# hbdat/cvpr22_cross_modal_pseudo_labeling

Hardware: AMD Instinct MI355X
Metric: images/sec student-teacher train step (COCO 800x1333) (higher is better)
Workload: dtype f32 (bf16x3 split MFMA, fp32 accum); 1 GPU; student_teacher_mask_rcnn_uncertainty.yaml R-50-C4, 2 img/GPU 3x800x1333, fwd+bwd+allreduce+SGD; global_batch=2, parallelism=dp1, losses_finite=True, pipelined=True

## Files before the change

cvpr22_cross_modal_pseudo_labeling_amd/_C.py:

```python
import contextlib
import functools
import ctypes
import threading

import torch

from . import _cpu, _lib

_L = _lib.load()


def _stream():
    return torch._C._cuda_getCurrentRawStream(torch.cuda.current_device())


class _Same:

    def __enter__(self):
        return None

    def __exit__(self, *exc):
        return False


# ... 652 lines not shown
        if not (pooled.is_cuda and pooled.dtype == torch.float32 and pooled.dim() == 2):
            raise RuntimeError("gate_split_pair: pooled must be a 2-D float32 HIP tensor")
        pooled = pooled.contiguous()
    if dy is not None:
        if not (dy.is_cuda and dy.dtype == torch.float32 and dy.dim() == 2):
            raise RuntimeError("gate_split_pair: 2-D float32 HIP tensor expected")
        if dy.stride(1) != 1 or dy.stride(0) % 4 or dy.data_ptr() % 16:
            dy = dy.contiguous()
        rows, cols = dy.shape
    else:
        rows, cols = pooled.shape[0] * pool_rows, pooled.shape[1]
    if pooled is not None and (pool_rows <= 0 or pooled.shape != (rows // max(pool_rows, 1), cols) or rows % pool_rows):
        raise RuntimeError("gate_split_pair: pooled must be [rows / pool_rows, cols]")
    dev = dy.device if dy is not None else pooled.device
    is_pair = 0
    if gate is not None:
        is_pair = int(gate.dtype == torch.bfloat16)
        if not (gate.is_cuda and gate.is_contiguous() and gate.shape == (rows, cols * (2 if is_pair else 1))
                and gate.dtype in (torch.bfloat16, torch.float32)):
            raise RuntimeError("gate_split_pair: gate must be the contiguous fp32 or pair form of the forward output")
    out = torch.empty((rows, 2 * cols), dtype=torch.bfloat16, device=dev)
    g32 = torch.empty((rows, cols), dtype=torch.float32, device=dev) if want_f32 else None
    if out.numel() == 0:
        return out, g32
    if selected is not None:
        selected, group_slot = _dev(selected, "selected"), _dev(group_slot, "group_slot", torch.int32)
        if pool_rows <= 0 or rows % pool_rows or selected.dim() != 2 or selected.shape[1] != cols or \
                selected.shape[0] % pool_rows or group_slot.numel() != rows // pool_rows:
            raise RuntimeError("gate_split_pair: selected must be [S * pool_rows, cols] and group_slot [rows / pool_rows]")
    with _on(dev):
        rc = _L.ovis_gate_split_pair_rows_f32(0 if dy is None else dy.data_ptr(), 0 if dy is None else dy.stride(0),
# ... 161 lines not shown
    if m == 0 or n == 0:
        return c, cp, pooled
    if bias is not None:
        bias = _dev(bias, "bias")
    with _on(dev):
        rc = _L.ovis_split_gemm_pair_rp_pool(a_pair.data_ptr(), 2 * a_pair.stride(0), b_pair.data_ptr(), 2 * b_pair.stride(0),
                                             0 if c is None else c.data_ptr(), n, 0 if cp is None else cp.data_ptr(), 4 * n,
                                             0 if bias is None else bias.data_ptr(),
                                             0 if residual_pair is None else residual_pair.data_ptr(),
                                             0 if residual_pair is None else 2 * residual_pair.stride(0), m, n, ch,
                                             int(bool(relu)), pooled.data_ptr(), int(pool_rows), 1.0 / pool_rows, _stream())
    _lib.check(rc, "split_gemm_pair_rp_pool")
    return c, cp, pooled


def weight_prep_pair(w, scale=None, want_transposed=False):
    if not (w.is_cuda and w.dtype == torch.float32 and w.dim() == 4):
        raise RuntimeError("weight_prep_pair: [N,C,KH,KW] float32 HIP tensor expected")
    w = w.detach().contiguous()
    n, c, kh, kw = w.shape
    t = kh * kw
    fwd = torch.empty((n, 2 * t * c), dtype=torch.bfloat16, device=w.device)
    bwd = torch.empty((c, 2 * t * n), dtype=torch.bfloat16, device=w.device) if want_transposed else None
    if scale is not None:
        scale = _dev(scale.detach(), "scale")
    with _on(w.device):
        rc = _L.ovis_weight_prep_pair_f32(w.data_ptr(), 0 if scale is None else scale.data_ptr(), fwd.data_ptr(),
                                          0 if bwd is None else bwd.data_ptr(), n, c, t, _stream())
    _lib.check(rc, "weight_prep_pair")
    return fwd, bwd
# ... 511 lines not shown
```

cvpr22_cross_modal_pseudo_labeling_amd/_lib.py:

```python
import ctypes
import os

_HERE = os.path.dirname(os.path.abspath(__file__))
LIB_PATH = os.path.join(_HERE, "libovis_hip.so")

OVIS_OK = 0
_ERRORS = {-1: "OVIS_EINVAL (bad size or null pointer)",
           -2: "OVIS_ENOSPC (workspace too small)",
           -3: "OVIS_ERANGE (problem size not supported by the kernel)"}

_vp, _i, _f, _sz, _l = ctypes.c_void_p, ctypes.c_int, ctypes.c_float, ctypes.c_size_t, ctypes.c_long

SIGNATURES = {
    "ovis_version": (ctypes.c_char_p, []),
    "ovis_roi_align_forward_f32": (_i, [_vp, _vp, _vp, _i, _i, _i, _i, _i, _i, _i, _f, _i, _vp]),
    "ovis_roi_align_forward_workspace_bytes": (_sz, [_i, _i, _i]),
    "ovis_roi_align_forward_mfma_supported": (_i, [_i, _i, _i, _i]),
    "ovis_roi_align_forward_ws_f32": (_i, [_vp, _vp, _vp, _i, _i, _i, _i, _i, _i, _i, _f, _i, _vp, _sz, _vp]),
    "ovis_roi_align_forward_strided_nhwc_f32": (_i, [_vp, _vp, _vp, _i, _i, _i, _i, _i, _i, _i, _i, _f, _i, _vp]),
    "ovis_roi_align_forward_strided_pair_f32": (_i, [_vp, _vp, _vp, _i, _i, _i, _i, _i, _i, _i, _i, _f, _i, _vp]),
    "ovis_roi_align_forward_strided_from_nhwc_f32": (_i, [_vp, _vp, _vp, _i, _i, _i, _i, _i, _i, _i, _i, _f, _i, _i, _vp]),
    "ovis_roi_align_backward_f32": (_i, [_vp, _vp, _vp, _i, _i, _i, _i, _i, _i, _i, _f, _i, _vp]),
    "ovis_roi_align_backward_workspace_bytes": (_sz, [_i, _i, _i, _i]),
    "ovis_roi_align_backward_plane_supported": (_i, [_i, _i, _i, _i]),
# ... 29 lines not shown
    "ovis_gate_split_pair_rows_f32": (_i, [_vp, _l, _vp, _i, _vp, _vp, _l, _i, _vp, _i, _vp, _vp, _vp]),
    "ovis_gate_split_pair_f32": (_i, [_vp, _l, _vp, _i, _vp, _vp, _l, _i, _vp, _i, _vp]),
    "ovis_im2col_nchw_pair_f32": (_i, [_vp, _vp] + [_i] * 9 + [_vp]),
    "ovis_weight_prep_pair_f32": (_i, [_vp, _vp, _vp, _vp, _i, _i, _i, _vp]),
    "ovis_slab_reduce_f32": (_i, [_vp, _vp, _vp, _i, _i, _i, _i, _vp]),
    "ovis_im2col_pair": (_i, [_vp, _vp, _l, _i, _i, _i, _i, _i, _vp]),
    "ovis_split_gemm_tn_slices": (_i, [_l, _i, _i, _i]),
    "ovis_split_gemm_pair_tn": (_i, [_vp, _l, _vp, _l, _vp, _i, _l, _i, _i, _i, _i, _i, _i, _vp]),
    "ovis_split_gemm_pair_gated": (_i, [_vp, _l, _vp, _l, _vp, _l, _vp, _l, _vp, _l, _l] + [_i] * 8 + [_vp]),
    "ovis_split_gemm_pair_gated_ws": (_i, [_vp, _l, _vp, _l, _vp, _l, _vp, _l, _vp, _l, _l] + [_i] * 7 + [_vp, _sz, _i, _vp]),
    "ovis_split_gemm_pair_workspace_bytes": (_sz, [_l, _i, _i, _i, _i, _i, _i]),
    "ovis_split_gemm_pair_workspace_bytes_ex": (_sz, [_l, _i, _i, _i, _i, _i, _i, _i]),
    "ovis_split_gemm_pair_rp_gated": (_i, [_vp, _l, _vp, _l, _vp, _l, _vp, _l, _vp, _l, _vp, _l, _l, _i, _i, _i, _vp]),
    "ovis_split_gemm_pair_pool_supported": (_i, [_l, _i, _i, _i]),
    "ovis_split_gemm_pair_rp_pool": (_i, [_vp, _l, _vp, _l, _vp, _l, _vp, _l, _vp, _vp, _l, _l, _i, _i, _i, _vp, _i, _f, _vp]),
    "ovis_split_gemm_pair_rp": (_i, [_vp, _l, _vp, _l, _vp, _l, _vp, _l, _vp, _vp, _l, _l, _i, _i, _i, _vp, _sz, _i, _vp]),
    "ovis_split_gemm_pair": (_i, [_vp, _l, _vp, _l, _vp, _l, _vp, _l, _vp, _l, _vp, _vp, _l, _l] + [_i] * 9
                             + [_vp, _sz, _i, _vp]),
    "ovis_match_encode_f32": (_i, [_vp, _vp, _vp, _i, _i, _f, _f, _i, _f, _f, _f, _f, _vp, _vp, _vp, _vp]),
    "ovis_rpn_match_encode_f32": (_i, [_vp, _vp, _vp, _i, _i, _f, _f, _i, _f, _f, _f, _f, _vp, _vp, _vp, _vp]),
    "ovis_project_masks_f32": (_i, [_vp, _vp, _vp, _i, _i, _i, _i, _i, _vp, _vp]),
    "ovis_gemm_f32": (_i, [_vp, _l, _l, _vp, _l, _l, _vp, _vp, _l, _i, _i, _i, _vp]),
    "ovis_gemm_ex_f32": (_i, [_vp, _l, _l, _vp, _l, _l, _vp, _i, _f, _i, _vp, _l, _i, _i, _i, _vp]),
    "ovis_gemm_f32_workspace_bytes": (_sz, [_i, _i, _i]),
    "ovis_gemm_ex_ws_f32": (_i, [_vp, _l, _l, _vp, _l, _l, _vp, _i, _f, _i, _vp, _l, _i, _i, _i, _vp, _sz, _vp]),
    "ovis_deform_im2col_f32": (_i, [_vp, _vp, _vp, _vp] + [_i] * 13 + [_vp]),
    "ovis_deform_col2im_f32": (_i, [_vp, _vp, _vp, _vp] + [_i] * 13 + [_vp]),
    "ovis_deform_col2im_coord_f32": (_i, [_vp, _vp, _vp, _vp, _vp, _vp] + [_i] * 13 + [_vp]),
    "ovis_deform_im2col_pair_rows_f32": (_i, [_vp, _vp, _vp, _vp, _l] + [_i] * 15 + [_vp]),
    "ovis_deform_col2im_rows_f32": (_i, [_vp, _l, _vp, _vp, _vp, _vp, _vp, _vp] + [_i] * 15 + [_vp]),
# ... 40 lines not shown
```

cvpr22_cross_modal_pseudo_labeling_amd/csrc/split_gemm.hip:

```cpp
#include <stdlib.h>

#include "ovis_common.h"
constexpr int kGroupWidth = 4;

namespace {
typedef short bf16x8 __attribute__((ext_vector_type(8)));
typedef float f32x4 __attribute__((ext_vector_type(4)));
typedef __bf16 b2 __attribute__((ext_vector_type(2)));
typedef float f2 __attribute__((ext_vector_type(2)));

__device__ char g_zero_line[128];

enum { PLAIN = 0, SHIFTED = 1, HALO = 2, DEFORM = 3 };
constexpr int kHalo = 8;

struct SplitGemmArgs {
  const char* A; long a_rs;
  const char* A2; long a2_rs;
  const char* B; long b_rs;
  float* C; long ldc;
  char* Cp; long cp_rs;
  const float* bias; const float* res; long ldr;
  const char* resp; long resp_rs;
  const char* gate; long gate_rs;
  float* pool; int pool_rows; float pool_scale;
  float* slab;
  long M; int N; int ch; int ch2; int T; int H; int W; int KH; int KW; int flip; int relu; int gw;
  int kslices; int steps_per_slice;
  const float* dimg; const float* doff; const float* dmask;
  int Ho; int Wo; int sh; int sw; int ph; int pw; int dlh; int dlw; int dg;
};

__device__ __forceinline__ void glds16(const char* gsrc, char* lds_wave_base) {
  __builtin_amdgcn_global_load_lds((const __attribute__((address_space(1))) void*)gsrc,
                                   (__attribute__((address_space(3))) void*)lds_wave_base, 16, 0, 0);
}

__device__ __forceinline__ unsigned pack_bf16(float a, float b) {
  f2 v = {a, b};
  return __builtin_bit_cast(unsigned, __builtin_convertvector(v, b2));
}

struct EpilogueOperands {
  uint2 a, b;
};

struct EpilogueSource {
  const char* base;
  long row_bytes;
  int second;
};

__device__ __forceinline__ EpilogueSource epilogue_source(const SplitGemmArgs& p) {
  EpilogueSource s;
  s.base = p.res ? (const char*)p.res : (p.resp ? p.resp : p.gate);
// ... 44 lines not shown
    *(uint2*)(d + 64) = make_uint2(l01, l23);
  }
  return v;
}

__device__ __forceinline__ void epilogue_store4(const SplitGemmArgs& p, long m, int n, f32x4 v) {
  const long poff = (long)(n >> 5) * 128 + (n & 31) * 2;
  f32x4 bias4 = {0.f, 0.f, 0.f, 0.f};
  if (p.bias) bias4 = *(const f32x4*)(p.bias + n);
  const EpilogueSource src = epilogue_source(p);
  EpilogueOperands o;
  if (src.base) epilogue_fetch4(src, m, epilogue_column_bytes(p, n, poff), o);
  epilogue_apply4(p, m, n, poff, v, bias4, o);
}

template <int WM, int WN, int MODE, int NS, int OCC, bool DUAL = false, bool POOL = false>
__global__ __launch_bounds__(WM * WN * 64, OCC) void split_gemm_kernel(SplitGemmArgs p, int tiles_n, int ntiles) {
  constexpr int BM = WM * 64, BN = WN * 64, NW = WM * WN;
  constexpr int A_ROWS = MODE == HALO ? BM + 2 * kHalo + 2 : BM;
  constexpr int ZROW = BM + 2 * kHalo;
  constexpr int A_BYTES = A_ROWS * 128, B_BYTES = BN * 128, STAGE = A_BYTES + B_BYTES;
  constexpr int A_PIECES = (MODE == HALO ? BM + 2 * kHalo : BM) / 8;
  constexpr int AI = (A_PIECES + NW - 1) / NW;
  constexpr int BI = BN / 8 / NW;
  static_assert(MODE != HALO || NS == 1, "the halo tile is single-staged");
  static_assert(NW * 4096 <= STAGE * NS, "epilogue staging fits the k-loop's LDS");
  extern __shared__ __attribute__((aligned(16))) char smem[];

  const int lane = threadIdx.x & 63, wave = __builtin_amdgcn_readfirstlane(threadIdx.x >> 6);
  int id;
  {
// ... 316 lines not shown
      const long m = m0 + wm * 64 + (piece >> 1) * 16 + ((piece & 1) * 2 + j) * 4 + er;
      const long mc = m < m_last ? m : m_last;
      epilogue_fetch4(src, mc, src_col, o[j]);
      if constexpr (DUAL) g[j] = *(const uint2*)(gate_col + mc * p.gate_rs);
    }
  };
  f32x4 ps0 = {0.f, 0.f, 0.f, 0.f}, ps1 = ps0, ps2 = ps0;
  int pool_b1 = 0, pool_b2 = 0;
  long pool_map0 = 0;
  if constexpr (POOL) {
    const long mw = m0 + wm * 64;
    pool_map0 = mw / p.pool_rows;
    pool_b1 = (int)((pool_map0 + 1) * p.pool_rows - mw);
    pool_b2 = pool_b1 + p.pool_rows;
  }
#pragma unroll
  for (int i = 0; i < NBUF - 1; ++i) fetch(i, ops[i], gates[i]);
#pragma unroll
  for (int f = 0; f < 4; ++f) {
#pragma unroll
    for (int g = 0; g < 4; ++g) *(f32x4*)(stg + frow * 256 + (((g * 4 + fc) ^ frow) << 4)) = acc[f][g];
#pragma unroll
    for (int h = 0; h < 2; ++h) {
      const int piece = f * 2 + h;
      if (piece + NBUF - 1 < 8) fetch(piece + NBUF - 1, ops[(piece + NBUF - 1) % NBUF], gates[(piece + NBUF - 1) % NBUF]);
#pragma unroll
      for (int j = 0; j < 2; ++j) {
        const int r = (h * 2 + j) * 4 + er;
        const f32x4 v = *(const f32x4*)(stg + r * 256 + ((es ^ r) << 4));
        const long m = m0 + wm * 64 + f * 16 + r;
        if (m < p.M && col_ok) {
          if (slab) *(f32x4*)(slab + m * p.N + n) = v;
          else {
            const f32x4 fin = epilogue_apply4<DUAL>(p, m, n, poff, v, bias4, ops[piece % NBUF][j], gates[piece % NBUF][j]);
            if constexpr (POOL) {
              const int rr = f * 16 + r;
              const f32x4 z = {0.f, 0.f, 0.f, 0.f};
              ps0 += rr < pool_b1 ? fin : z;
              ps1 += (rr >= pool_b1 && rr < pool_b2) ? fin : z;
              ps2 += rr >= pool_b2 ? fin : z;
            }
          }
        }
      }
    }
  }
  if constexpr (POOL) {
    f32x4* ps[3] = {&ps0, &ps1, &ps2};
#pragma unroll
    for (int sgm = 0; sgm < 3; ++sgm) {
      f32x4 v = *ps[sgm];
#pragma unroll
      for (int e = 0; e < 4; ++e) {
        v[e] += __shfl_xor(v[e], 16, 64);
        v[e] += __shfl_xor(v[e], 32, 64);
      }
      const long first = (m0 + wm * 64) + (sgm == 0 ? 0 : (sgm == 1 ? pool_b1 : pool_b2));
// ... 233 lines not shown
    const long r = i / oc;
    const int c = (int)(i - r * oc) * 8;
    const float4 v0 = *(const float4*)(src + r * src_rs + c), v1 = *(const float4*)(src + r * src_rs + c + 4);
    const unsigned h0 = pack_bf16(v0.x, v0.y), h1 = pack_bf16(v0.z, v0.w), h2 = pack_bf16(v1.x, v1.y),
                   h3 = pack_bf16(v1.z, v1.w);
    const unsigned l0 = pack_bf16(v0.x - __uint_as_float(h0 << 16), v0.y - __uint_as_float(h0 & 0xffff0000u));
    const unsigned l1 = pack_bf16(v0.z - __uint_as_float(h1 << 16), v0.w - __uint_as_float(h1 & 0xffff0000u));
    const unsigned l2 = pack_bf16(v1.x - __uint_as_float(h2 << 16), v1.y - __uint_as_float(h2 & 0xffff0000u));
    const unsigned l3 = pack_bf16(v1.z - __uint_as_float(h3 << 16), v1.w - __uint_as_float(h3 & 0xffff0000u));
    char* d = dst + r * 4L * cols + (long)(c >> 5) * 128 + (c & 31) * 2;
    *(uint4*)d = make_uint4(h0, h1, h2, h3);
    *(uint4*)(d + 64) = make_uint4(l0, l1, l2, l3);
  }
}

template <bool GATE_PAIR, bool WRITE_F32>
__global__ __launch_bounds__(256) void gate_split_pair_kernel(const float* __restrict__ dy, long dy_rs,
                                                             const void* __restrict__ gate, char* __restrict__ dst,
                                                             float* __restrict__ g32, long rows, int cols,
                                                             const float* __restrict__ gpool, int pool_rows,
                                                             float pool_scale, const float* __restrict__ gsel,
                                                             const int* __restrict__ group_slot) {
  const int oc = cols >> 3;
  const long total = rows * oc;
  for (long i = (long)blockIdx.x * 256 + threadIdx.x; i < total; i += (long)gridDim.x * 256) {
    const long r = i / oc;
    const int c = (int)(i - r * oc) * 8;
    float v[8];
    if (dy) {
      *(float4*)v = *(const float4*)(dy + r * dy_rs + c);
      *(float4*)(v + 4) = *(const float4*)(dy + r * dy_rs + c + 4);
// ... 11 lines not shown
    }
    if (gsel) {
      const long grp = r / pool_rows;
      const int slot = group_slot[grp];
      if (slot >= 0) {
        const float* gs = gsel + ((long)slot * pool_rows + (r - grp * pool_rows)) * cols + c;
        float q[8];
        *(float4*)q = *(const float4*)gs;
        *(float4*)(q + 4) = *(const float4*)(gs + 4);
#pragma unroll
        for (int k = 0; k < 8; ++k) v[k] += q[k];
      }
    }
    const long poff = r * 4L * cols + (long)(c >> 5) * 128 + (c & 31) * 2;
    if (gate) {
      if (GATE_PAIR) {
        const uint4 h = *(const uint4*)((const char*)gate + poff);
        const unsigned w[4] = {h.x, h.y, h.z, h.w};
#pragma unroll
        for (int k = 0; k < 4; ++k) {
          const unsigned a = w[k] & 0xffffu, b = w[k] >> 16;
          if (a == 0u || a >= 0x8000u) v[2 * k] = 0.f;
          if (b == 0u || b >= 0x8000u) v[2 * k + 1] = 0.f;
        }
      } else {
        float y[8];
        *(float4*)y = *(const float4*)((const float*)gate + r * (long)cols + c);
        *(float4*)(y + 4) = *(const float4*)((const float*)gate + r * (long)cols + c + 4);
#pragma unroll
        for (int k = 0; k < 8; ++k)
          if (!(y[k] > 0.f)) v[k] = 0.f;
// ... 169 lines not shown
                                       pool_rows, nullptr, nullptr, stream);
}

extern "C" int ovis_gate_split_pair_rows_f32(const float* dy, long dy_row_stride, const void* gate, int gate_is_pair,
                                             void* dst_pair, float* g_f32, long rows, int cols, const float* g_pooled,
                                             int pool_rows, const float* g_selected, const int32_t* group_slot,
                                             void* stream) {
  if (rows < 0 || cols < 0) return OVIS_EINVAL;
  if (rows == 0 || cols == 0) return OVIS_OK;
  if ((!dy && !g_pooled && !g_selected) || !dst_pair || ((g_pooled || g_selected) && (pool_rows <= 0 || rows % pool_rows != 0)) ||
      ((g_selected != nullptr) != (group_slot != nullptr)))
    return OVIS_EINVAL;
  if (cols % 32 != 0 || dy_row_stride % 4 != 0 || ((uintptr_t)dy & 15) || ((uintptr_t)dst_pair & 15) ||
      ((uintptr_t)gate & 15) || ((uintptr_t)g_f32 & 15) || ((uintptr_t)g_pooled & 15) || ((uintptr_t)g_selected & 15))
    return OVIS_ERANGE;
  const float pool_scale = g_pooled ? 1.f / (float)pool_rows : 0.f;
  const long total = rows * (cols / 8);
  const long blocks = (total + 255) / 256;
  const unsigned grid = (unsigned)(blocks < 8L * OVIS_NUM_CU ? blocks : 8L * OVIS_NUM_CU);
  hipStream_t s = (hipStream_t)stream;
#define OVIS_GS(GP_, WF_)                                                                                          \
  hipLaunchKernelGGL((gate_split_pair_kernel<GP_, WF_>), dim3(grid), dim3(256), 0, s, dy, dy_row_stride, gate,      \
                     (char*)dst_pair, g_f32, rows, cols, g_pooled, pool_rows, pool_scale, g_selected, group_slot)
  if (gate_is_pair) { if (g_f32) OVIS_GS(true, true); else OVIS_GS(true, false); }
  else { if (g_f32) OVIS_GS(false, true); else OVIS_GS(false, false); }
#undef OVIS_GS
  OVIS_LAUNCH_CHECK();
  return OVIS_OK;
}

extern "C" int ovis_im2col_nchw_pair_f32(const float* src, void* dst_pair, int num, int channels, int height,
                                         int width, int kh, int kw, int stride, int pad, int k_padded, void* stream) {
  if (num < 0 || channels <= 0 || height <= 0 || width <= 0 || kh <= 0 || kw <= 0 || stride <= 0 || pad < 0)
    return OVIS_EINVAL;
  if (num == 0) return OVIS_OK;
  if (!src || !dst_pair) return OVIS_EINVAL;
  if (k_padded % 32 != 0 || k_padded < kh * kw * channels || ((uintptr_t)dst_pair & 15)) return OVIS_ERANGE;
  const int ho = (height + 2 * pad - kh) / stride + 1, wo = (width + 2 * pad - kw) / stride + 1;
  if (ho <= 0 || wo <= 0) return OVIS_EINVAL;
  const long total = (long)num * ho * wo * (k_padded / 8);
// ... 215 lines not shown
  return q.kslices > 1 ? (size_t)q.kslices * (size_t)m * (size_t)n * sizeof(float) : 0;
}

extern "C" size_t ovis_split_gemm_pair_workspace_bytes(long m, int n, int channels, int channels2, int taps_h,
                                                       int taps_w, int width) {
  return ovis_split_gemm_pair_workspace_bytes_ex(m, n, channels, channels2, taps_h, taps_w, width, 0);
}

static int split_gemm_pair_impl(const void* a_pair, long a_row_bytes, const void* a2_pair, long a2_row_bytes,
                                const void* b_pair, long b_row_bytes, float* c, long ldc, void* c_pair,
                                long c_pair_row_bytes, const float* bias, const float* residual, long ldr,
                                const void* residual_pair, long residual_pair_row_bytes,
                                const void* gate_pair, long gate_row_bytes, long m, int n, int channels, int channels2,
                                int taps_h, int taps_w, int height, int width, int flip, int relu, void* workspace,
                                size_t workspace_bytes, int config, void* stream, float* pool = nullptr, int pool_rows = 0,
                                float pool_scale = 1.f) {
  if (m < 0 || n < 0 || channels < 0 || channels2 < 0 || taps_h <= 0 || taps_w <= 0 || !(taps_h & 1) || !(taps_w & 1))
    return OVIS_EINVAL;
  if (m == 0 || n == 0) return OVIS_OK;
  if (!a_pair || !b_pair || (!c && !c_pair && !pool) || channels == 0 || m > 0x7fffff00L) return OVIS_EINVAL;
  if (pool && (pool_rows < 32 || pool_rows > 64 || ((uintptr_t)pool & 15))) return OVIS_ERANGE;
  const int T = taps_h * taps_w;
  if (T > 1 && (height <= 0 || width <= 0 || height > 32767 || width > 32767 || channels2 != 0)) return OVIS_EINVAL;
  if (channels2 != 0 && !a2_pair) return OVIS_EINVAL;
  const bool dual = residual_pair && gate_pair && !residual;
  if (!dual && (residual != nullptr) + (residual_pair != nullptr) + (gate_pair != nullptr) > 1) return OVIS_EINVAL;
  if (dual && T > 1) return OVIS_ERANGE;
  if (channels % 32 != 0 || channels2 % 32 != 0 || n % 4 != 0 || (c_pair && n % 32 != 0) || a_row_bytes % 16 != 0 ||
      a2_row_bytes % 16 != 0 || b_row_bytes % 16 != 0 || ((uintptr_t)a_pair & 15) || ((uintptr_t)a2_pair & 15) ||
      ((uintptr_t)b_pair & 15) || ((uintptr_t)c & 15) || ((uintptr_t)c_pair & 15) || ((uintptr_t)bias & 15) ||
      ((uintptr_t)residual & 15) || ((uintptr_t)workspace & 15) || ldc % 4 != 0 || ldr % 4 != 0 ||
      c_pair_row_bytes % 16 != 0)
    return OVIS_ERANGE;
  if (config < 0 || config > 0x1ffff) return OVIS_ERANGE;
  SplitGemmPlan q = split_gemm_plan(m, n, channels, channels2, taps_h, taps_w, width, config);
  if (q.kslices > 1 && (!workspace || workspace_bytes < (size_t)q.kslices * (size_t)m * (size_t)n * sizeof(float))) {
    q = split_gemm_plan(m, n, channels, channels2, taps_h, taps_w, width, config | 8);
  }
  SplitGemmArgs p;
  p.A = (const char*)a_pair; p.a_rs = a_row_bytes;
  p.A2 = (const char*)a2_pair; p.a2_rs = a2_row_bytes;
  p.B = (const char*)b_pair; p.b_rs = b_row_bytes;
  p.C = c; p.ldc = ldc; p.Cp = (char*)c_pair; p.cp_rs = c_pair_row_bytes;
  p.bias = bias; p.res = residual; p.ldr = ldr;
  p.resp = (const char*)residual_pair; p.resp_rs = residual_pair_row_bytes;
  p.gate = (const char*)gate_pair; p.gate_rs = gate_row_bytes;
  p.slab = q.kslices > 1 ? (float*)workspace : nullptr;
  p.pool = pool; p.pool_rows = pool_rows; p.pool_scale = pool_scale;
  p.M = m; p.N = n; p.ch = channels; p.ch2 = channels2; p.T = T; p.H = height; p.W = width; p.KH = taps_h; p.KW = taps_w;
  p.flip = flip; p.relu = relu;
  p.kslices = q.kslices; p.steps_per_slice = q.steps_per_slice;
  p.gw = (q.tiles_n % kGroupWidth == 0) ? kGroupWidth : (q.tiles_n % 4 == 0) ? 4 : q.tiles_n;
  const long ntiles = (long)q.tiles_m * q.tiles_n;
  const long nblocks = ntiles * q.kslices;
  if (nblocks > 0x7fffffffL) return OVIS_ERANGE;
  hipStream_t s = (hipStream_t)stream;
#define OVIS_SG_LAUNCH__(WM_, WN_, MODE_, NS_, OCC_, DUAL_, POOL_)                                                   \
  do {                                                                                                              \
    constexpr int a_rows = MODE_ == HALO ? WM_ * 64 + 2 * kHalo + 2 : WM_ * 64;                                      \
    constexpr int lds = NS_ * (a_rows * 128 + WN_ * 64 * 128);                                                       \
    static bool attr_set = false;                                                                                   \
    if (!attr_set) {                                                                                                \
      OVIS_HIP_TRY(hipFuncSetAttribute((const void*)split_gemm_kernel<WM_, WN_, MODE_, NS_, OCC_, DUAL_, POOL_>,    \
                                       hipFuncAttributeMaxDynamicSharedMemorySize, lds));                           \
      attr_set = true;                                                                                              \
    }                                                                                                               \
    hipLaunchKernelGGL((split_gemm_kernel<WM_, WN_, MODE_, NS_, OCC_, DUAL_, POOL_>), dim3((unsigned)nblocks),      \
                       dim3(WM_ * WN_ * 64), lds, s, p, q.tiles_n, (int)ntiles);                                    \
  } while (0)
#define OVIS_SG_LAUNCH_(WM_, WN_, MODE_, NS_, OCC_, DUAL_) OVIS_SG_LAUNCH__(WM_, WN_, MODE_, NS_, OCC_, DUAL_, false)
#define OVIS_SG_LAUNCH(WM_, WN_, MODE_, NS_, OCC_) OVIS_SG_LAUNCH_(WM_, WN_, MODE_, NS_, OCC_, false)
  if (pool) {
    if (dual || q.narrow || q.mode != PLAIN || q.kslices > 1) return OVIS_ERANGE;
    if (q.stages == 1) OVIS_SG_LAUNCH__(2, 2, PLAIN, 1, 4, false, true); else OVIS_SG_LAUNCH__(2, 2, PLAIN, 2, 2, false, true);
  } else if (dual) {
    if (q.narrow || q.mode != PLAIN || q.kslices > 1) return OVIS_ERANGE;
    if (q.stages == 1) OVIS_SG_LAUNCH_(2, 2, PLAIN, 1, 4, true); else OVIS_SG_LAUNCH_(2, 2, PLAIN, 2, 2, true);
  } else if (q.narrow) {
    if (q.mode == PLAIN) OVIS_SG_LAUNCH(2, 1, PLAIN, 1, 2); else OVIS_SG_LAUNCH(2, 1, SHIFTED, 1, 2);
  } else if (q.mode == HALO) {
    OVIS_SG_LAUNCH(2, 2, HALO, 1, 4);
  } else if (q.mode == SHIFTED) {
    if (q.stages == 1) OVIS_SG_LAUNCH(2, 2, SHIFTED, 1, 4); else OVIS_SG_LAUNCH(2, 2, SHIFTED, 2, 2);
  } else {
    if (q.stages == 1) OVIS_SG_LAUNCH(2, 2, PLAIN, 1, 4); else OVIS_SG_LAUNCH(2, 2, PLAIN, 2, 2);
  }
#undef OVIS_SG_LAUNCH__
#undef OVIS_SG_LAUNCH_
#undef OVIS_SG_LAUNCH
  OVIS_LAUNCH_CHECK();
  if (q.kslices > 1) {
    p.slab = (float*)workspace;
    const long total = m * (n / 4);
    const long blocks = (total + 255) / 256;
    const unsigned grid = (unsigned)(blocks < 8L * OVIS_NUM_CU ? blocks : 8L * OVIS_NUM_CU);
    hipLaunchKernelGGL(split_gemm_finish_kernel, dim3(grid), dim3(256), 0, s, p);
    OVIS_LAUNCH_CHECK();
  }
  return OVIS_OK;
}

// ... 23 lines not shown
  if (m <= 0 || n <= 0 || channels <= 0 || channels % 32 || n % 32 || pool_rows < 32 || pool_rows > 64) return 0;
  const SplitGemmPlan q = split_gemm_plan(m, n, channels, 0, 1, 1, 0, 0);
  return !q.narrow && q.mode == PLAIN && q.kslices == 1;
}

extern "C" int ovis_split_gemm_pair_rp_pool(const void* a_pair, long a_row_bytes, const void* b_pair, long b_row_bytes,
                                            float* c, long ldc, void* c_pair, long c_pair_row_bytes, const float* bias,
                                            const void* residual_pair, long residual_pair_row_bytes, long m, int n,
                                            int channels, int relu, float* pooled, int pool_rows, float pool_scale,
                                            void* stream) {
  if (!pooled) return OVIS_EINVAL;
  if (n % 32 != 0 || (residual_pair && (residual_pair_row_bytes % 16 != 0 || ((uintptr_t)residual_pair & 15)))) return OVIS_ERANGE;
  return split_gemm_pair_impl(a_pair, a_row_bytes, nullptr, 0, b_pair, b_row_bytes, c, ldc, c_pair, c_pair_row_bytes, bias,
                              nullptr, 0, residual_pair, residual_pair_row_bytes, nullptr, 0, m, n, channels, 0, 1, 1, 0, 0,
                              0, relu, nullptr, 0, 8, stream, pooled, pool_rows, pool_scale);
}

extern "C" int ovis_split_gemm_pair_gated(const void* a_pair, long a_row_bytes, const void* b_pair, long b_row_bytes,
                                          float* c, long ldc, void* c_pair, long c_pair_row_bytes,
                                          const void* gate_pair, long gate_row_bytes, long m, int n, int channels,
                                          int taps_h, int taps_w, int height, int width, int flip, int config,
                                          void* stream) {
  if (!gate_pair || gate_row_bytes % 16 != 0 || ((uintptr_t)gate_pair & 15) || n % 32 != 0) return OVIS_ERANGE;
  return split_gemm_pair_impl(a_pair, a_row_bytes, nullptr, 0, b_pair, b_row_bytes, c, ldc, c_pair, c_pair_row_bytes,
                              nullptr, nullptr, 0, nullptr, 0, gate_pair, gate_row_bytes, m, n, channels, 0, taps_h, taps_w,
                              height, width, flip, 0, nullptr, 0, config | 8, stream);
}

extern "C" int ovis_split_gemm_pair_gated_ws(const void* a_pair, long a_row_bytes, const void* b_pair, long b_row_bytes,
                                             float* c, long ldc, void* c_pair, long c_pair_row_bytes,
// ... 66 lines not shown
```

cvpr22_cross_modal_pseudo_labeling_amd/layers/pair_bottleneck.py:

```python
import torch
from torch.autograd import Function
from torch.autograd.function import once_differentiable

from .. import _C


def pair_weight(w2d):
    return _C.split_pair(w2d.contiguous())


def conv_weight_matrix(w):
    n, c, kh, kw = w.shape
    return w.permute(0, 2, 3, 1).reshape(n, kh * kw * c)


def conv_weight_matrix_t(w):
    n, c, kh, kw = w.shape
    return w.permute(1, 2, 3, 0).reshape(c, kh * kw * n)


def dw_pair(gp, xp, conv=None):
    n, k = gp.shape[1] // 2, xp.shape[1] // 2
    if _C.split_gemm_pair_tn_supported(n, k, conv):
        return _C.split_gemm_pair_tn(gp, xp, conv)
# ... 1 lines not shown
        xp = _C.im2col_pair(xp, *conv)
        k = xp.shape[1] // 2
    q = torch.mm(gp.t(), xp, out_dtype=torch.float32)
    return q.view(n // 32, 2, 32, k // 32, 2, 32).sum(dim=(1, 4)).reshape(n, k)


def _dw(gp, xp, w, scale, conv=None):
    n, c = w.shape[0], w.shape[1]
    if _C.split_gemm_pair_tn_supported(n, c, conv):
        return _C.split_gemm_pair_tn(gp, xp, conv, scale=scale, weight_shape=tuple(w.shape))
    d = dw_pair(gp, xp, conv).view(n, w.shape[2], w.shape[3], c).permute(0, 3, 1, 2)
    return d if scale is None else d * scale.view(-1, 1, 1, 1)


ONE_CALL_BACKWARD_ROWS = 40000

_WEIGHTS_EPOCH = [0]


def note_weights_written():
    _WEIGHTS_EPOCH[0] += 1


class WeightPrepPlan:

    def __init__(self, blocks):
        import numpy as np
        tile = _C.weight_prep_tile()
        self.max_taps = 1
        self.entries = {}
# ... 121 lines not shown
            wpairs = {"w1": p1, "w2": p2, "w3": p3, "wd": pd}
            wts = (t1, t2, t3, td)
        elif need_bwd:
            wts = wpairs.get("wts")
        f32 = bool(want_f32 or pool or not want_pair)
        x_real = x is not None and not is_placeholder(x)
        _, o1p = _C.split_gemm_pair(xp, wpairs["w1"], b1, None, True, False, True)
        _, o2p = _C.split_gemm_pair(o1p, wpairs["w2"], b2, None, True, False, True, conv=(h, w, kh, kw, False))
        if wd is not None:
            w3d = wpairs.get("w3d")
            if w3d is None:
                w3d = torch.cat([wpairs["w3"], wpairs["wd"]], 1)
            out, outp = _C.split_gemm_pair(o2p, w3d, b3, None, True, f32, want_pair, a2_pair=xp)
        elif x_real:
            out, outp = _C.split_gemm_pair(o2p, wpairs["w3"], b3, x, True, f32, want_pair)
        pooled_k = None
        if wd is None and not x_real:
            fused_pool = (pool and 32 <= h * w <= 64
                          and _C.split_gemm_pair_pool_supported(o2p.shape[0], wpairs["w3"].shape[0], o2p.shape[1] // 2, h * w))
            if fused_pool:
                keep = need_bwd or want_pair or select is not None or not pool_only_ok
                out, outp, pooled_k = _C.split_gemm_pair_rp_pool(o2p, wpairs["w3"], b3, xp, True, keep, want_pair, h * w)
                if out is None and outp is None:
                    out = nan_placeholder(pooled_k.device, o2p.shape[0], pooled_k.shape[1])
            else:
                out, outp = _C.split_gemm_pair(o2p, wpairs["w3"], b3, None, True, f32, want_pair, residual_pair=xp)
        if pooled_k is not None:
            pooled = pooled_k
        else:
            pooled = out.view(-1, h * w, out.shape[1]).mean(dim=1) if pool else None
        out_sel = out.view(-1, h * w, out.shape[1]).index_select(0, select) if (select is not None and f32) else None
        gate_src = out if out is not None else outp
        if out is None:
            out = nan_placeholder(outp.device, outp.shape[0], outp.shape[1] // 2)
        ctx.save_for_backward(xp, o1p, o2p, gate_src, w1, w2, w3, wd, s1, s2, s3, sd, select if out_sel is not None else None)
        ctx.wts = wts
        ctx.geom = (h, w, kh, kw)
        ctx.link_in = link_in if (wd is None and not x_real) else None
        ctx.link_out = link_out if not f32 else None
        ctx.set_materialize_grads(False)
        if outp is not None:
            ctx.mark_non_differentiable(outp)
        return out, outp, pooled, out_sel

    @staticmethod
    @once_differentiable
    def backward(ctx, dout, _dpair, dpooled, dsel):
# ... 128 lines not shown
```

include/ovis_hip.h:

```cpp
#ifndef OVIS_HIP_H_
#define OVIS_HIP_H_

#include <stddef.h>
#include <stdint.h>

#ifdef __cplusplus
extern "C" {
#endif

#define OVIS_OK 0
#define OVIS_EINVAL (-1)
#define OVIS_ENOSPC (-2)
#define OVIS_ERANGE (-3)

const char* ovis_version(void);

int ovis_roi_align_forward_f32(const float* input, const float* rois, float* output,
                               int num_rois, int batch, int channels, int height,
                               int width, int pooled_h, int pooled_w,
                               float spatial_scale, int sampling_ratio, void* stream);

size_t ovis_roi_align_forward_workspace_bytes(int num_rois, int height, int width);
int ovis_roi_align_forward_mfma_supported(int height, int width, int pooled_h, int pooled_w);
int ovis_roi_align_forward_ws_f32(const float* input, const float* rois, float* output,
// ... 254 lines not shown
int ovis_deform_im2col_pair_rows_f32(const float* input_nhwc, const float* offset, const float* mask, void* columns_pair,
                                     long columns_row_bytes, int batch, int channels, int height, int width, int out_h,
                                     int out_w, int kernel_h, int kernel_w, int stride_h, int stride_w, int pad_h, int pad_w,
                                     int dil_h, int dil_w, int deformable_group, void* stream);
int ovis_deform_col2im_rows_f32(const float* dcol_rows, long dcol_ld, const float* input_nhwc, const float* offset,
                                const float* mask, float* grad_input_nhwc, float* grad_offset, float* grad_mask, int batch,
                                int channels, int height, int width, int out_h, int out_w, int kernel_h, int kernel_w,
                                int stride_h, int stride_w, int pad_h, int pad_w, int dil_h, int dil_w, int deformable_group,
                                void* stream);

int ovis_split_gemm_pair_pool_supported(long m, int n, int channels, int pool_rows);
int ovis_split_gemm_pair_rp_pool(const void* a_pair, long a_row_bytes, const void* b_pair, long b_row_bytes, float* c,
                                 long ldc, void* c_pair, long c_pair_row_bytes, const float* bias,
                                 const void* residual_pair, long residual_pair_row_bytes, long m, int n, int channels,
                                 int relu, float* pooled, int pool_rows, float pool_scale, void* stream);

int ovis_sgd_momentum_multi_f32(const void* items, const void* blocks, int num_blocks, float lr, float weight_decay,
                                float momentum, int apply_weight_decay, void* stream);
int ovis_sgd_chunk_elements(void);

size_t ovis_bottleneck_identity_backward_workspace_bytes(long m, int channels, int mid_channels, int taps_h, int taps_w,
                                                         int width, int config);
int ovis_bottleneck_identity_backward(
    const void* g3_pair, long g3_row_bytes, const void* x_pair, long x_row_bytes, const void* o1_pair, long o1_row_bytes,
    const void* o2_pair, long o2_row_bytes, const void* t1_pair, long t1_row_bytes, const void* t2_pair, long t2_row_bytes,
    const void* t3_pair, long t3_row_bytes, const float* scale1, const float* scale2, const float* scale3, long m, int channels,
    int mid_channels, int taps_h, int taps_w, int height, int width, void* g2_pair, void* g1_pair, void* gx_pair, float* dw1,
    float* dw2, float* dw3, void* workspace, size_t workspace_bytes, int config, void* stream, void* side_stream);

int ovis_weight_prep_pair_multi_f32(const void* items, const void* blocks, int num_blocks, int max_taps, void* stream);
// ... 7 lines not shown
```

Before: 60.68 images/sec.

## Save a bit-packed ReLU mask and selected rows from fused pooled GEMM epilogue

In the last bottleneck block's fused GEMM+pool path, the epilogue now emits a 1-bit-per-element ReLU mask built with wave ballots, plus the ROI-selected output rows, instead of a full fp32 output. Backward uses the int64 mask as the gate in gate_split_pair. This removes the large fp32 activation write, its later read, and the separate index_select. The cost is extra ballot and packing work and scattered selected-row stores in the epilogue, plus a new kernel template instantiation.

After: 60.71 images/sec (median of 4 runs). Within noise of the previous version (+0.0%).

```diff
diff --git a/cvpr22_cross_modal_pseudo_labeling_amd/_C.py b/cvpr22_cross_modal_pseudo_labeling_amd/_C.py
--- a/cvpr22_cross_modal_pseudo_labeling_amd/_C.py
+++ b/cvpr22_cross_modal_pseudo_labeling_amd/_C.py
@@ -690,7 +690,11 @@
         raise RuntimeError("gate_split_pair: pooled must be [rows / pool_rows, cols]")
     dev = dy.device if dy is not None else pooled.device
     is_pair = 0
-    if gate is not None:
+    if gate is not None and gate.dtype == torch.int64:
+        is_pair = 2
+        if not (gate.is_cuda and gate.is_contiguous() and cols % 64 == 0 and gate.shape == (rows, cols // 64)):
+            raise RuntimeError("gate_split_pair: a mask gate must be the contiguous [rows, cols / 64] int64 ReLU mask")
+    elif gate is not None:
         is_pair = int(gate.dtype == torch.bfloat16)
         if not (gate.is_cuda and gate.is_contiguous() and gate.shape == (rows, cols * (2 if is_pair else 1))
                 and gate.dtype in (torch.bfloat16, torch.float32)):
@@ -882,6 +886,40 @@
     return c, cp, pooled
 
 
+def split_gemm_pair_rp_pool_masked(a_pair, b_pair, bias, residual_pair, relu, out_pair, pool_rows, mask_kind, group_slot=None,
+                                   num_selected=0):
+    for t, name in ((a_pair, "a_pair"), (b_pair, "b_pair")) + (((residual_pair, "residual_pair"),) if residual_pair is not None else ()):
+        if not (t.is_cuda and t.dtype == torch.bfloat16 and t.dim() == 2 and t.stride(1) == 1):
+            raise RuntimeError(f"split_gemm_pair_rp_pool_masked: {name} must be a 2-D bfloat16 HIP tensor in pair layout")
+    m, ch = a_pair.shape[0], a_pair.shape[1] // 2
+    n, k = b_pair.shape[0], b_pair.shape[1] // 2
+    if k != ch or m % pool_rows or n % 64 or (residual_pair is not None and residual_pair.shape != (m, 2 * n)):
+        raise RuntimeError("split_gemm_pair_rp_pool_masked: shape mismatch")
+    dev = a_pair.device
+    cp = torch.empty((m, 2 * n), dtype=torch.bfloat16, device=dev) if out_pair else None
+    pooled = torch.zeros((m // pool_rows, n), dtype=torch.float32, device=dev)
+    mask = torch.empty((m, n // 64), dtype=torch.int64, device=dev)
+    sel = None
+    if group_slot is not None:
+        group_slot = _dev(group_slot, "group_slot", torch.int32)
+        if group_slot.numel() != m // pool_rows:
+            raise RuntimeError("split_gemm_pair_rp_pool_masked: group_slot must be [M / pool_rows]")
+        sel = torch.empty((num_selected, pool_rows, n), dtype=torch.float32, device=dev)
+    if m == 0 or n == 0:
+        return cp, pooled, mask, sel
+    if bias is not None:
+        bias = _dev(bias, "bias")
+    with _on(dev):
+        rc = _L.ovis_split_gemm_pair_rp_pool_masked(
+            a_pair.data_ptr(), 2 * a_pair.stride(0), b_pair.data_ptr(), 2 * b_pair.stride(0),
+            0 if cp is None else cp.data_ptr(), 4 * n, 0 if bias is None else bias.data_ptr(),
+            0 if residual_pair is None else residual_pair.data_ptr(), 0 if residual_pair is None else 2 * residual_pair.stride(0),
+            m, n, ch, int(bool(relu)), pooled.data_ptr(), int(pool_rows), 1.0 / pool_rows, mask.data_ptr(), int(mask_kind),
+            0 if sel is None else sel.data_ptr(), 0 if group_slot is None else group_slot.data_ptr(), _stream())
+    _lib.check(rc, "split_gemm_pair_rp_pool_masked")
+    return cp, pooled, mask, sel
+
+
 def weight_prep_pair(w, scale=None, want_transposed=False):
     if not (w.is_cuda and w.dtype == torch.float32 and w.dim() == 4):
         raise RuntimeError("weight_prep_pair: [N,C,KH,KW] float32 HIP tensor expected")
diff --git a/cvpr22_cross_modal_pseudo_labeling_amd/_lib.py b/cvpr22_cross_modal_pseudo_labeling_amd/_lib.py
--- a/cvpr22_cross_modal_pseudo_labeling_amd/_lib.py
+++ b/cvpr22_cross_modal_pseudo_labeling_amd/_lib.py
@@ -67,6 +67,8 @@
     "ovis_split_gemm_pair_rp_gated": (_i, [_vp, _l, _vp, _l, _vp, _l, _vp, _l, _vp, _l, _vp, _l, _l, _i, _i, _i, _vp]),
     "ovis_split_gemm_pair_pool_supported": (_i, [_l, _i, _i, _i]),
     "ovis_split_gemm_pair_rp_pool": (_i, [_vp, _l, _vp, _l, _vp, _l, _vp, _l, _vp, _vp, _l, _l, _i, _i, _i, _vp, _i, _f, _vp]),
+    "ovis_split_gemm_pair_rp_pool_masked": (_i, [_vp, _l, _vp, _l, _vp, _l, _vp, _vp, _l, _l, _i, _i, _i, _vp, _i, _f, _vp, _i,
+                                                 _vp, _vp, _vp]),
     "ovis_split_gemm_pair_rp": (_i, [_vp, _l, _vp, _l, _vp, _l, _vp, _l, _vp, _vp, _l, _l, _i, _i, _i, _vp, _sz, _i, _vp]),
     "ovis_split_gemm_pair": (_i, [_vp, _l, _vp, _l, _vp, _l, _vp, _l, _vp, _l, _vp, _vp, _l, _l] + [_i] * 9
                              + [_vp, _sz, _i, _vp]),
diff --git a/cvpr22_cross_modal_pseudo_labeling_amd/csrc/split_gemm.hip b/cvpr22_cross_modal_pseudo_labeling_amd/csrc/split_gemm.hip
--- a/cvpr22_cross_modal_pseudo_labeling_amd/csrc/split_gemm.hip
+++ b/cvpr22_cross_modal_pseudo_labeling_amd/csrc/split_gemm.hip
@@ -29,6 +29,8 @@
   int kslices; int steps_per_slice;
   const float* dimg; const float* doff; const float* dmask;
   int Ho; int Wo; int sh; int sw; int ph; int pw; int dlh; int dlw; int dg;
+  unsigned long long* mask = nullptr; int mask_kind = 0;
+  float* sel = nullptr; const int* sel_slot = nullptr;
 };
 
 __device__ __forceinline__ void glds16(const char* gsrc, char* lds_wave_base) {
@@ -39,6 +41,16 @@
 __device__ __forceinline__ unsigned pack_bf16(float a, float b) {
   f2 v = {a, b};
   return __builtin_bit_cast(unsigned, __builtin_convertvector(v, b2));
+}
+
+__device__ __forceinline__ int relu_mask_bit(int c) { return ((c & 3) << 4) | ((c & 63) >> 2); }
+
+__device__ __forceinline__ unsigned relu_mask_bits4(int kind, f32x4 v) {
+  if (kind == 0) return (v.x > 0.f ? 1u : 0u) | (v.y > 0.f ? 2u : 0u) | (v.z > 0.f ? 4u : 0u) | (v.w > 0.f ? 8u : 0u);
+  const unsigned h01 = pack_bf16(v.x, v.y), h23 = pack_bf16(v.z, v.w);
+  const unsigned a0 = h01 & 0xffffu, a1 = h01 >> 16, a2 = h23 & 0xffffu, a3 = h23 >> 16;
+  return (a0 - 1u < 0x7fffu ? 1u : 0u) | (a1 - 1u < 0x7fffu ? 2u : 0u) | (a2 - 1u < 0x7fffu ? 4u : 0u) |
+         (a3 - 1u < 0x7fffu ? 8u : 0u);
 }
 
 struct EpilogueOperands {
@@ -113,7 +125,7 @@
   epilogue_apply4(p, m, n, poff, v, bias4, o);
 }
 
-template <int WM, int WN, int MODE, int NS, int OCC, bool DUAL = false, bool POOL = false>
+template <int WM, int WN, int MODE, int NS, int OCC, bool DUAL = false, bool POOL = false, bool MASK = false>
 __global__ __launch_bounds__(WM * WN * 64, OCC) void split_gemm_kernel(SplitGemmArgs p, int tiles_n, int ntiles) {
   constexpr int BM = WM * 64, BN = WN * 64, NW = WM * WN;
   constexpr int A_ROWS = MODE == HALO ? BM + 2 * kHalo + 2 : BM;
@@ -460,6 +472,17 @@
     pool_b1 = (int)((pool_map0 + 1) * p.pool_rows - mw);
     pool_b2 = pool_b1 + p.pool_rows;
   }
+  int sel_s0 = -1, sel_s1 = -1, sel_s2 = -1;
+  unsigned long long* const mask_col = MASK ? p.mask + ((n0 + wn * 64) >> 6) : nullptr;
+  const long mask_rs = p.N >> 6;
+  if constexpr (POOL && MASK) {
+    if (p.sel) {
+      const long groups = p.M / p.pool_rows;
+      if (pool_map0 < groups) sel_s0 = p.sel_slot[pool_map0];
+      if (pool_map0 + 1 < groups) sel_s1 = p.sel_slot[pool_map0 + 1];
+      if (pool_map0 + 2 < groups) sel_s2 = p.sel_slot[pool_map0 + 2];
+    }
+  }
 #pragma unroll
   for (int i = 0; i < NBUF - 1; ++i) fetch(i, ops[i], gates[i]);
 #pragma unroll
@@ -475,6 +498,7 @@
         const int r = (h * 2 + j) * 4 + er;
         const f32x4 v = *(const f32x4*)(stg + r * 256 + ((es ^ r) << 4));
         const long m = m0 + wm * 64 + f * 16 + r;
+        unsigned mbits = 0u;
         if (m < p.M && col_ok) {
           if (slab) *(f32x4*)(slab + m * p.N + n) = v;
           else {
@@ -485,8 +509,23 @@
               ps0 += rr < pool_b1 ? fin : z;
               ps1 += (rr >= pool_b1 && rr < pool_b2) ? fin : z;
               ps2 += rr >= pool_b2 ? fin : z;
+              if constexpr (MASK) {
+                const int sg = rr < pool_b1 ? 0 : (rr < pool_b2 ? 1 : 2);
+                const int slot = sg == 0 ? sel_s0 : (sg == 1 ? sel_s1 : sel_s2);
+                if (slot >= 0)
+                  *(f32x4*)(p.sel + (long)(slot * p.pool_rows + (int)(m - (pool_map0 + sg) * p.pool_rows)) * p.N + n) = fin;
+              }
             }
+            if constexpr (MASK) mbits = relu_mask_bits4(p.mask_kind, fin);
           }
+        }
+        if constexpr (MASK) {
+          const int sh = er * 16;
+          const unsigned long long b0 = __ballot(mbits & 1u), b1 = __ballot(mbits & 2u), b2 = __ballot(mbits & 4u),
+                                   b3 = __ballot(mbits & 8u);
+          const unsigned long long word = ((b0 >> sh) & 0xffffull) | (((b1 >> sh) & 0xffffull) << 16) |
+                                          (((b2 >> sh) & 0xffffull) << 32) | (((b3 >> sh) & 0xffffull) << 48);
+          if (es == 0 && m < p.M && col_ok) mask_col[m * mask_rs] = word;
         }
       }
     }
@@ -750,7 +789,7 @@
   }
 }
 
-template <bool GATE_PAIR, bool WRITE_F32>
+template <int GATE, bool WRITE_F32>
 __global__ __launch_bounds__(256) void gate_split_pair_kernel(const float* __restrict__ dy, long dy_rs,
                                                              const void* __restrict__ gate, char* __restrict__ dst,
                                                              float* __restrict__ g32, long rows, int cols,
@@ -792,7 +831,12 @@
     }
     const long poff = r * 4L * cols + (long)(c >> 5) * 128 + (c & 31) * 2;
     if (gate) {
-      if (GATE_PAIR) {
+      if (GATE == 2) {
+        const unsigned long long mw = *((const unsigned long long*)gate + r * (long)(cols >> 6) + (c >> 6));
+#pragma unroll
+        for (int k = 0; k < 8; ++k)
+          if (!((mw >> relu_mask_bit(c + k)) & 1ull)) v[k] = 0.f;
+      } else if (GATE == 1) {
         const uint4 h = *(const uint4*)((const char*)gate + poff);
         const unsigned w[4] = {h.x, h.y, h.z, h.w};
 #pragma unroll
@@ -992,6 +1036,7 @@
   if (cols % 32 != 0 || dy_row_stride % 4 != 0 || ((uintptr_t)dy & 15) || ((uintptr_t)dst_pair & 15) ||
       ((uintptr_t)gate & 15) || ((uintptr_t)g_f32 & 15) || ((uintptr_t)g_pooled & 15) || ((uintptr_t)g_selected & 15))
     return OVIS_ERANGE;
+  if (gate_is_pair == 2 && cols % 64 != 0) return OVIS_ERANGE;
   const float pool_scale = g_pooled ? 1.f / (float)pool_rows : 0.f;
   const long total = rows * (cols / 8);
   const long blocks = (total + 255) / 256;
@@ -1000,8 +1045,9 @@
 #define OVIS_GS(GP_, WF_)                                                                                          \
   hipLaunchKernelGGL((gate_split_pair_kernel<GP_, WF_>), dim3(grid), dim3(256), 0, s, dy, dy_row_stride, gate,      \
                      (char*)dst_pair, g_f32, rows, cols, g_pooled, pool_rows, pool_scale, g_selected, group_slot)
-  if (gate_is_pair) { if (g_f32) OVIS_GS(true, true); else OVIS_GS(true, false); }
-  else { if (g_f32) OVIS_GS(false, true); else OVIS_GS(false, false); }
+  if (gate_is_pair == 2) { if (g_f32) OVIS_GS(2, true); else OVIS_GS(2, false); }
+  else if (gate_is_pair) { if (g_f32) OVIS_GS(1, true); else OVIS_GS(1, false); }
+  else { if (g_f32) OVIS_GS(0, true); else OVIS_GS(0, false); }
 #undef OVIS_GS
   OVIS_LAUNCH_CHECK();
   return OVIS_OK;
@@ -1247,7 +1293,8 @@
                                 const void* gate_pair, long gate_row_bytes, long m, int n, int channels, int channels2,
                                 int taps_h, int taps_w, int height, int width, int flip, int relu, void* workspace,
                                 size_t workspace_bytes, int config, void* stream, float* pool = nullptr, int pool_rows = 0,
-                                float pool_scale = 1.f) {
+                                float pool_scale = 1.f, unsigned long long* mask = nullptr, int mask_kind = 0,
+                                float* sel = nullptr, const int* sel_slot = nullptr) {
   if (m < 0 || n < 0 || channels < 0 || channels2 < 0 || taps_h <= 0 || taps_w <= 0 || !(taps_h & 1) || !(taps_w & 1))
     return OVIS_EINVAL;
   if (m == 0 || n == 0) return OVIS_OK;
@@ -1266,6 +1313,10 @@
       c_pair_row_bytes % 16 != 0)
     return OVIS_ERANGE;
   if (config < 0 || config > 0x1ffff) return OVIS_ERANGE;
+  if (mask && (n % 64 != 0 || ((uintptr_t)mask & 7) || mask_kind < 0 || mask_kind > 1)) return OVIS_ERANGE;
+  if ((sel != nullptr) != (sel_slot != nullptr) || (sel && (!pool || !mask || m % pool_rows != 0 || ((uintptr_t)sel & 15))))
+    return OVIS_EINVAL;
+  if (mask) config |= 8;
   SplitGemmPlan q = split_gemm_plan(m, n, channels, channels2, taps_h, taps_w, width, config);
   if (q.kslices > 1 && (!workspace || workspace_bytes < (size_t)q.kslices * (size_t)m * (size_t)n * sizeof(float))) {
     q = split_gemm_plan(m, n, channels, channels2, taps_h, taps_w, width, config | 8);
@@ -1280,6 +1331,7 @@
   p.gate = (const char*)gate_pair; p.gate_rs = gate_row_bytes;
   p.slab = q.kslices > 1 ? (float*)workspace : nullptr;
   p.pool = pool; p.pool_rows = pool_rows; p.pool_scale = pool_scale;
+  p.mask = mask; p.mask_kind = mask_kind; p.sel = sel; p.sel_slot = sel_slot;
   p.M = m; p.N = n; p.ch = channels; p.ch2 = channels2; p.T = T; p.H = height; p.W = width; p.KH = taps_h; p.KW = taps_w;
   p.flip = flip; p.relu = relu;
   p.kslices = q.kslices; p.steps_per_slice = q.steps_per_slice;
@@ -1288,24 +1340,31 @@
   const long nblocks = ntiles * q.kslices;
   if (nblocks > 0x7fffffffL) return OVIS_ERANGE;
   hipStream_t s = (hipStream_t)stream;
-#define OVIS_SG_LAUNCH__(WM_, WN_, MODE_, NS_, OCC_, DUAL_, POOL_)                                                   \
+#define OVIS_SG_LAUNCH_M(WM_, WN_, MODE_, NS_, OCC_, DUAL_, POOL_, MASK_)                                           \
   do {                                                                                                              \
     constexpr int a_rows = MODE_ == HALO ? WM_ * 64 + 2 * kHalo + 2 : WM_ * 64;                                      \
     constexpr int lds = NS_ * (a_rows * 128 + WN_ * 64 * 128);                                                       \
     static bool attr_set = false;                                                                                   \
     if (!attr_set) {                                                                                                \
-      OVIS_HIP_TRY(hipFuncSetAttribute((const void*)split_gemm_kernel<WM_, WN_, MODE_, NS_, OCC_, DUAL_, POOL_>,    \
+      OVIS_HIP_TRY(hipFuncSetAttribute((const void*)split_gemm_kernel<WM_, WN_, MODE_, NS_, OCC_, DUAL_, POOL_, MASK_>, \
                                        hipFuncAttributeMaxDynamicSharedMemorySize, lds));                           \
       attr_set = true;                                                                                              \
     }                                                                                                               \
-    hipLaunchKernelGGL((split_gemm_kernel<WM_, WN_, MODE_, NS_, OCC_, DUAL_, POOL_>), dim3((unsigned)nblocks),      \
+    hipLaunchKernelGGL((split_gemm_kernel<WM_, WN_, MODE_, NS_, OCC_, DUAL_, POOL_, MASK_>), dim3((unsigned)nblocks), \
                        dim3(WM_ * WN_ * 64), lds, s, p, q.tiles_n, (int)ntiles);                                    \
   } while (0)
+#define OVIS_SG_LAUNCH__(WM_, WN_, MODE_, NS_, OCC_, DUAL_, POOL_) OVIS_SG_LAUNCH_M(WM_, WN_, MODE_, NS_, OCC_, DUAL_, POOL_, false)
 #define OVIS_SG_LAUNCH_(WM_, WN_, MODE_, NS_, OCC_, DUAL_) OVIS_SG_LAUNCH__(WM_, WN_, MODE_, NS_, OCC_, DUAL_, false)
 #define OVIS_SG_LAUNCH(WM_, WN_, MODE_, NS_, OCC_) OVIS_SG_LAUNCH_(WM_, WN_, MODE_, NS_, OCC_, false)
   if (pool) {
     if (dual || q.narrow || q.mode != PLAIN || q.kslices > 1) return OVIS_ERANGE;
-    if (q.stages == 1) OVIS_SG_LAUNCH__(2, 2, PLAIN, 1, 4, false, true); else OVIS_SG_LAUNCH__(2, 2, PLAIN, 2, 2, false, true);
+    if (mask) {
+      if (q.stages == 1) OVIS_SG_LAUNCH_M(2, 2, PLAIN, 1, 4, false, true, true); else OVIS_SG_LAUNCH_M(2, 2, PLAIN, 2, 2, false, true, true);
+    } else {
+      if (q.stages == 1) OVIS_SG_LAUNCH__(2, 2, PLAIN, 1, 4, false, true); else OVIS_SG_LAUNCH__(2, 2, PLAIN, 2, 2, false, true);
+    }
+  } else if (mask) {
+    return OVIS_ERANGE;
   } else if (dual) {
     if (q.narrow || q.mode != PLAIN || q.kslices > 1) return OVIS_ERANGE;
     if (q.stages == 1) OVIS_SG_LAUNCH_(2, 2, PLAIN, 1, 4, true); else OVIS_SG_LAUNCH_(2, 2, PLAIN, 2, 2, true);
@@ -1318,6 +1377,7 @@
   } else {
     if (q.stages == 1) OVIS_SG_LAUNCH(2, 2, PLAIN, 1, 4); else OVIS_SG_LAUNCH(2, 2, PLAIN, 2, 2);
   }
+#undef OVIS_SG_LAUNCH_M
 #undef OVIS_SG_LAUNCH__
 #undef OVIS_SG_LAUNCH_
 #undef OVIS_SG_LAUNCH
@@ -1371,6 +1431,20 @@
   return split_gemm_pair_impl(a_pair, a_row_bytes, nullptr, 0, b_pair, b_row_bytes, c, ldc, c_pair, c_pair_row_bytes, bias,
                               nullptr, 0, residual_pair, residual_pair_row_bytes, nullptr, 0, m, n, channels, 0, 1, 1, 0, 0,
                               0, relu, nullptr, 0, 8, stream, pooled, pool_rows, pool_scale);
+}
+
+extern "C" int ovis_split_gemm_pair_rp_pool_masked(const void* a_pair, long a_row_bytes, const void* b_pair,
+                                                   long b_row_bytes, void* c_pair, long c_pair_row_bytes, const float* bias,
+                                                   const void* residual_pair, long residual_pair_row_bytes, long m, int n,
+                                                   int channels, int relu, float* pooled, int pool_rows, float pool_scale,
+                                                   void* mask, int mask_kind, float* selected, const int32_t* group_slot,
+                                                   void* stream) {
+  if (!pooled || !mask) return OVIS_EINVAL;
+  if (n % 64 != 0 || (residual_pair && (residual_pair_row_bytes % 16 != 0 || ((uintptr_t)residual_pair & 15)))) return OVIS_ERANGE;
+  return split_gemm_pair_impl(a_pair, a_row_bytes, nullptr, 0, b_pair, b_row_bytes, nullptr, 0, c_pair, c_pair_row_bytes, bias,
+                              nullptr, 0, residual_pair, residual_pair_row_bytes, nullptr, 0, m, n, channels, 0, 1, 1, 0, 0,
+                              0, relu, nullptr, 0, 8, stream, pooled, pool_rows, pool_scale, (unsigned long long*)mask,
+                              mask_kind, selected, group_slot);
 }
 
 extern "C" int ovis_split_gemm_pair_gated(const void* a_pair, long a_row_bytes, const void* b_pair, long b_row_bytes,
diff --git a/cvpr22_cross_modal_pseudo_labeling_amd/layers/pair_bottleneck.py b/cvpr22_cross_modal_pseudo_labeling_amd/layers/pair_bottleneck.py
--- a/cvpr22_cross_modal_pseudo_labeling_amd/layers/pair_bottleneck.py
+++ b/cvpr22_cross_modal_pseudo_labeling_amd/layers/pair_bottleneck.py
@@ -39,6 +39,8 @@
 
 
 ONE_CALL_BACKWARD_ROWS = 40000
+
+RELU_MASK_LAST_BLOCK = True
 
 _WEIGHTS_EPOCH = [0]
 
@@ -190,23 +192,32 @@
             out, outp = _C.split_gemm_pair(o2p, w3d, b3, None, True, f32, want_pair, a2_pair=xp)
         elif x_real:
             out, outp = _C.split_gemm_pair(o2p, wpairs["w3"], b3, x, True, f32, want_pair)
-        pooled_k = None
+        pooled_k = relu_mask = out_sel = None
         if wd is None and not x_real:
             fused_pool = (pool and 32 <= h * w <= 64
                           and _C.split_gemm_pair_pool_supported(o2p.shape[0], wpairs["w3"].shape[0], o2p.shape[1] // 2, h * w))
             if fused_pool:
                 keep = need_bwd or want_pair or select is not None or not pool_only_ok
-                out, outp, pooled_k = _C.split_gemm_pair_rp_pool(o2p, wpairs["w3"], b3, xp, True, keep, want_pair, h * w)
-                if out is None and outp is None:
-                    out = nan_placeholder(pooled_k.device, o2p.shape[0], pooled_k.shape[1])
+                n3 = wpairs["w3"].shape[0]
+                if RELU_MASK_LAST_BLOCK and need_bwd and select is not None and n3 % 64 == 0:
+                    slot = torch.full((o2p.shape[0] // (h * w),), -1, dtype=torch.int32, device=o2p.device)
+                    slot[select] = torch.arange(select.numel(), dtype=torch.int32, device=o2p.device)
+                    outp, pooled_k, relu_mask, out_sel = _C.split_gemm_pair_rp_pool_masked(
+                        o2p, wpairs["w3"], b3, xp, True, want_pair, h * w, 0, slot, select.numel())
+                    out = nan_placeholder(pooled_k.device, o2p.shape[0], n3)
+                else:
+                    out, outp, pooled_k = _C.split_gemm_pair_rp_pool(o2p, wpairs["w3"], b3, xp, True, keep, want_pair, h * w)
+                    if out is None and outp is None:
+                        out = nan_placeholder(pooled_k.device, o2p.shape[0], pooled_k.shape[1])
             else:
                 out, outp = _C.split_gemm_pair(o2p, wpairs["w3"], b3, None, True, f32, want_pair, residual_pair=xp)
         if pooled_k is not None:
             pooled = pooled_k
         else:
             pooled = out.view(-1, h * w, out.shape[1]).mean(dim=1) if pool else None
-        out_sel = out.view(-1, h * w, out.shape[1]).index_select(0, select) if (select is not None and f32) else None
-        gate_src = out if out is not None else outp
+        if relu_mask is None:
+            out_sel = out.view(-1, h * w, out.shape[1]).index_select(0, select) if (select is not None and f32) else None
+        gate_src = relu_mask if relu_mask is not None else (out if out is not None else outp)
         if out is None:
             out = nan_placeholder(outp.device, outp.shape[0], outp.shape[1] // 2)
         ctx.save_for_backward(xp, o1p, o2p, gate_src, w1, w2, w3, wd, s1, s2, s3, sd, select if out_sel is not None else None)
diff --git a/include/ovis_hip.h b/include/ovis_hip.h
--- a/include/ovis_hip.h
+++ b/include/ovis_hip.h
@@ -292,6 +292,11 @@
                                  long ldc, void* c_pair, long c_pair_row_bytes, const float* bias,
                                  const void* residual_pair, long residual_pair_row_bytes, long m, int n, int channels,
                                  int relu, float* pooled, int pool_rows, float pool_scale, void* stream);
+int ovis_split_gemm_pair_rp_pool_masked(const void* a_pair, long a_row_bytes, const void* b_pair, long b_row_bytes,
+                                        void* c_pair, long c_pair_row_bytes, const float* bias, const void* residual_pair,
+                                        long residual_pair_row_bytes, long m, int n, int channels, int relu, float* pooled,
+                                        int pool_rows, float pool_scale, void* mask, int mask_kind, float* selected,
+                                        const int32_t* group_slot, void* stream);
 
 int ovis_sgd_momentum_multi_f32(const void* items, const void* blocks, int num_blocks, float lr, float weight_decay,
                                 float momentum, int apply_weight_decay, void* stream);
```
